# ddiazdom/grlBWT

Measured on AMD Instinct MI355X. Metric: input MB/s building BCR BWT on 10 GB DNA reads, 1/2/4/8 MI355X, higher is better.
Workload: dtype u8; 1 GPU; 66225166 x 150 bp Illumina-style reads (10000000066 bytes) from a 330000000 bp genome, 0.5% substitutions; BASELINE configs[3]; input_resident=HBM, output=.rl_bwt image in HBM, parallelism=1 GPU

## Files before the change

grlbwt_amd/csrc/engine_impl.hpp:

```cpp

#include "switches.hpp"

namespace GRL_NS {

using prim::u8;
using prim::u16;
using prim::u32;
using prim::u64;
typedef GRL_IDX_T idx_t;

template <class T>
struct DBuf {
    T *p = nullptr;
    u64 n = 0;
    DBuf() {}
    explicit DBuf(u64 n_) { alloc(n_); }
    DBuf(const DBuf &) = delete;
    DBuf &operator=(const DBuf &) = delete;
    DBuf(DBuf &&o) noexcept : p(o.p), n(o.n) { o.p = nullptr; o.n = 0; }
    DBuf &operator=(DBuf &&o) noexcept {
        if (this != &o) { release(); p = o.p; n = o.n; o.p = nullptr; o.n = 0; }
        return *this;
    }
    ~DBuf() { release(); }
// ... 1631 lines not shown
static inline void build_rankbits32(RankBits &rb, const u32 *pos, u64 count, u64 nbits, const char *name) {
    u64 nw = nbits / 64 + 2;
    rb.words.alloc(nw);
    rb.base.alloc(nw + 1);
    rb.words.zero();
    prim::for_each((count + 15) / 16, BuildBits32Fn{pos, count, rb.words.p}, name);
    prim::exclusive_scan_nosync<idx_t>(nw, PopcIn{rb.words.p}, rb.base.p, true, name);
}

template <class L>
struct IdxIn {
    const L *p;
    GRL_DEV idx_t operator()(u64 i) const { return (idx_t)p[i]; }
};
struct SymHeadIn64 {
    const u32 *s;
    GRL_DEV u64 operator()(u64 t) const { return (t == 0 || s[t] != s[t - 1]) ? 1ull : 0ull; }
};
struct IdxIn64 {
    const idx_t *p;
    GRL_DEV u64 operator()(u64 i) const { return (u64)p[i]; }
};
struct PtrU32In {
    const u32 *p;
    GRL_DEV u32 operator()(u64 i) const { return p[i]; }
};
typedef prim::Pair<idx_t, idx_t> HeadLen;
struct HeadLenIn {
    const u32 *s; const idx_t *len;
    GRL_DEV HeadLen operator()(u64 t) const { return HeadLen((t == 0 || s[t] != s[t - 1]) ? (idx_t)1 : (idx_t)0, len[t]); }
};
struct DiffFn {
    const idx_t *start; idx_t *len;
    GRL_DEV void operator()(u64 r) const { len[r] = start[r + 1] - start[r]; }
};

struct Runs {
    DBuf<u32> sym;
    DBuf<idx_t> len;
    DBuf<idx_t> pos;
    u64 R = 0;
    u64 n = 0;
};
struct RunLen {
    const idx_t *len; const idx_t *pos;
    GRL_DEV idx_t operator()(u64 i) const { return len ? len[i] : (idx_t)(pos[i + 1] - pos[i]); }
};
struct RunLenIn64 {
    RunLen l;
    GRL_DEV u64 operator()(u64 i) const { return (u64)l(i); }
};

struct MergeEmitFn {
    static constexpr bool kWaveEmit = false;
    const u32 *sym; u64 n;
    u32 *osym; idx_t *ostart; u32 *map;
    GRL_DEV void operator()(u64 t, HeadLen ex, HeadLen v) const {
        if (v.a) { osym[ex.a] = sym[t]; ostart[ex.a] = ex.b; }
        if (t == n - 1) ostart[ex.a + v.a] = ex.b + v.b;
        if (map) map[t] = (u32)(ex.a + v.a - 1);
    }
};
static inline Runs merge_runs(const u32 *sym, const idx_t *len, u64 n, u32 *merged_index = nullptr) {
    Runs out;
    if (n == 0) { out.sym.alloc(0); out.len.alloc(0); return out; }
    DBuf<u32> hsym(n);
    DBuf<idx_t> ostart(n + 1);
    HeadLen tot = prim::exclusive_scan_emit<HeadLen>(n, HeadLenIn{sym, len}, MergeEmitFn{sym, n, hsym.p, ostart.p, merged_index}, "merge_runs.scan");
    u64 R = (u64)tot.a;
    out.n = (u64)tot.b;
    out.len.alloc(R);
    prim::for_each(R, DiffFn{ostart.p, out.len.p}, "merge_runs.len");
    if (R * 2 >= n) out.sym = std::move(hsym);
    else { out.sym.alloc(R); prim::d2d(out.sym.p, hsym.p, R * sizeof(u32)); }
    out.pos = std::move(ostart);
    out.R = R;
    return out;
}

struct CellSymFn {
    const u32 *t; u32 *sym; idx_t *len;
    GRL_DEV void operator()(u64 i) const { sym[i] = t[i] >> 2; len[i] = 1; }
};

template <class F>
struct StoreFn {
    F f; idx_t *out;
    GRL_DEV void operator()(u64 i) const { out[i] = f(i); }
};

struct PackGrammarFn {
    const u32 *g0; const u32 *g1; const u8 *has_hocc; u64 *gp;
    GRL_DEV void operator()(u64 u) const { gp[u] = ((u64)g1[u] << 32) | (u64)(g0[u] | (has_hocc[u] ? 0x80000000u : 0u)); }
};
struct ChainCountFn {
    const u32 *nsym; const u64 *gp; u32 sigma3;
    GRL_DEV idx_t operator()(u64 i) const {
        u64 c0 = gp[nsym[i]];
        idx_t c = (c0 & 0x80000000ull) ? 1 : 0;
        u32 nx = (u32)(c0 >> 32);
        while (nx >= sigma3) { c++; nx = (u32)(gp[nx - sigma3] >> 32); }
        return c;
    }
};
struct TakeCountIn {
    const u32 *nsym; const u64 *gp;
    GRL_DEV u64 operator()(u64 i) const { return (gp[nsym[i]] & 0x80000000ull) ? 1ull : 0ull; }
};
enum { CELLS_SEPARATE = 0, CELLS_PACKED = 1, CELLS_FUSED = 2 };
template <int MODE>
struct ChainExpandFn {
    const u32 *nsym; RunLen nlen; const u64 *gp; const idx_t *eoff;
    u32 sigma3, take_code;
    u32 *ekey; idx_t *eidx; u32 *esym; idx_t *elen; u64 *epack; u32 *term;
    int kb, lb;
    GRL_DEV void put(u64 e, u32 key, u32 sym, idx_t f) const {
        if (MODE == CELLS_FUSED) { epack[e] = ((u64)sym << (kb + lb)) | ((u64)f << kb) | (u64)key; return; }
        ekey[e] = key;
        if (MODE == CELLS_PACKED) epack[e] = ((u64)sym << 32) | (u64)f;
        else { eidx[e] = (idx_t)e; esym[e] = sym; elen[e] = f; }
    }
    GRL_DEV void operator()(u64 i) const {
        u32 cur = nsym[i];
        idx_t f = nlen(i);
        u64 e = eoff[i];
        u64 c = gp[cur];
        if (c & 0x80000000ull) put(e++, cur, take_code, f);
        u32 nx = (u32)(c >> 32);
        while (nx >= sigma3) {
            u32 b = nx - sigma3;
            put(e++, b, (u32)c & 0x7FFFFFFFu, f);
            c = gp[b];
            nx = (u32)(c >> 32);
        }
        term[i] = nx;
    }
};
struct ChainGen {
    const u32 *nsym; RunLen nlen; const u64 *gp;
    u32 sigma3, take_code;
    u32 *term;
    int kb, lb;
    GRL_DEV u32 start(u64 i) const { return nsym[i]; }
    GRL_DEV u64 node(u32 u) const { return gp[u]; }
    GRL_DEV bool owns(u64 rec) const { return (rec & 0x80000000ull) != 0; }
    GRL_DEV bool more(u64 rec) const { return (u32)(rec >> 32) >= sigma3; }
    GRL_DEV u32 next(u64 rec) const { return (u32)(rec >> 32) - sigma3; }
    GRL_DEV u64 item_bits(u64 i) const { return (u64)nlen(i) << kb; }
    GRL_DEV u64 key_own(u32 u, u64 ib) const { return ((u64)take_code << (kb + lb)) | ib | (u64)u; }
    GRL_DEV u64 key_step(u64 rec, u32 b, u64 ib) const { return ((u64)((u32)rec & 0x7FFFFFFFu) << (kb + lb)) | ib | (u64)b; }
    GRL_DEV void finish(u64 i, u64 rec) const { term[i] = (u32)(rec >> 32); }
};
struct NarrowCellFn {
    const u64 *in; u32 *out;
    GRL_DEV void operator()(u64 i) const { out[i] = (u32)in[i]; }
};
struct GatherCellFn {
    const idx_t *perm; const u32 *esym; const idx_t *elen; u32 *ssym; idx_t *slen;
    GRL_DEV void operator()(u64 t) const { u64 e = perm[t]; ssym[t] = esym[e]; slen[t] = elen[e]; }
};

struct NotCodeIn {
    const u32 *sym; u32 code;
    GRL_DEV idx_t operator()(u64 i) const { return sym[i] != code ? (idx_t)1 : (idx_t)0; }
};
struct CellView {
// ... 1274 lines not shown
        std::vector<u64> bh = bound.to_host(2 * ((u64)N + 1));
        cnt.assign(N, 0);
        for (int d = 0; d < N; d++) cnt[d] = bh[2 * (d + 1)] - bh[2 * d];
        if (res) rec = std::move(rec2);
    }
    template <class A, class F>
    void owner_round_trip(const Comm &C, const u64 *dsb, DBuf<u64> &req, u64 n, DBuf<A> &back, F answer, const char *name, const char *xname, DBuf<u32> *own_of = nullptr) {
        std::vector<u64> scnt(C.size, 0);
        try { bucket_by_owner(C, dsb, req, n, scnt, name, own_of); }
        catch (const prim::Error &e) { C.fail(e); std::fill(scnt.begin(), scnt.end(), 0); }
        const auto cn = C.counts(scnt);
        const std::vector<u64> &rcnt = cn.rcnt;
        const u64 nr = cn.total, maxb = cn.maxb;
        DBuf<u64> mine;
        DBuf<A> ans;
        try { mine.alloc(nr); ans.alloc(nr); back.alloc(n); } catch (const prim::Error &e) { C.fail(e); }
        C.allgather_u64({});
        C.named(xname).alltoall(req.p, scnt, mine.p, rcnt, 8, maxb);
        try { answer(mine.p, nr, ans.p); } catch (const prim::Error &e) { C.fail(e); }
        C.allgather_u64({});
        C.named(xname).alltoall(ans.p, rcnt, back.p, scnt, sizeof(A), maxb);
    }

    template <class cell_t, bool FIRST>
    struct DictIn {
        const Comm *C = nullptr;
        const cell_t *t = nullptr; CellOps<cell_t, FIRST> ops{};
        u64 D = 0, S = 0; u32 maxlen = 0, sigma = 0;
        const u64 *ph_pos = nullptr; const idx_t *ph_freq = nullptr; const u32 *ph_off = nullptr; const u8 *ph_lastT = nullptr;
        const u32 *fused_ph_slot = nullptr; u32 *fused_slot_val = nullptr;
        const prim::U128 *pkeys = nullptr; u64 pDs = 0; int pkb = 0;
        u32 pslot0 = 0;
        const std::vector<u64> *dbase = nullptr;
        const std::vector<u64> *sbase = nullptr;
        bool sharded_dict = false;
        u64 maxfreq = ~0ull;
    };
    struct SortKeyShape { int b, K, rb, kbits; u64 sent; };
    static SortKeyShape sort_key_shape(u32 sigma, u32 maxlen, int rb) {
        SortKeyShape s;
        s.b = std::max((int)bitlen64(sigma), 1); s.K = std::min(std::max((64 - rb) / s.b, 1), 16);
        const int kmax = prim::sw().sort_kmax;
        if (kmax >= 1 && s.K > kmax) s.K = kmax;
        if ((u64)s.K > (u64)maxlen + 1) s.K = (int)maxlen + 1;
        s.rb = (rb && s.K * s.b + rb > 64) ? 0 : rb;
        s.kbits = s.K * s.b + s.rb;
        s.sent = ((1ull << s.b) - 1ull) << s.rb;
        return s;
    }
    static void key_records_by_owner(const SufKeep &keep, const u32 *dict_sym, u64 q0, u64 nq, const SortKeyShape &ks, const RunKeys &rk, const u64 *dspl, int N,
                              u32 pos_base, const idx_t *ph_freq, u32 bwt_code, DBuf<u64> &sk, DBuf<u32> &sp, DBuf<u64> *sr, std::vector<u64> &scnt) {
        DBuf<u32> kex(nq + 1);
        const u64 nk = prim::exclusive_scan<u32>(nq, KeepRangeIn{keep, q0}, kex.p, false, "suffix_keep");
        DBuf<u64> lk(nk), bound(2 * ((u64)N + 1));
        DBuf<u32> lp(nk), own(nk), own2(nk), idx(nk), idx2(nk);
        DBuf<u64> lr;
        if (sr) lr.alloc(nk);
        prim::for_each(nq, KeyRangeFn{keep, kex.p, q0, dict_sym, ks.K, ks.b, dspl, N, lk.p, lp.p, own.p, idx.p, rk, pos_base,
                                      sr ? lr.p : nullptr, ph_freq, bwt_code}, "suffix_keys0");
        const int obits = std::max((int)bitlen64((u64)N - 1), 1);
        const int res = prim::sort_pairs<u32, u32>(own.p, idx.p, own2.p, idx2.p, nk, 0, obits, "dist.key_owner_sort");
        sk.alloc(nk); sp.alloc(nk);
        prim::for_each(nk, GatherKeyPosFn{res ? idx2.p : idx.p, lk.p, lp.p, sk.p, sp.p}, "dist.key_owner_sort");
        if (sr) { sr->alloc(nk); prim::for_each(nk, GatherU64Fn{res ? idx2.p : idx.p, lr.p, sr->p}, "dist.key_owner_sort"); }
        prim::for_each((u64)N + 1, KeyBoundFn{res ? own2.p : own.p, nk, nullptr, bound.p}, "dist.owner_bounds");
        std::vector<u64> bh = bound.to_host(2 * ((u64)N + 1));
        for (int d = 0; d < N; d++) scnt[d] = bh[2 * (d + 1)] - bh[2 * d];
    }
    static void first_sort_and_flags(DBuf<u64> &ka, DBuf<u32> &perm, u64 Sg, const SortKeyShape &ks, const RunKeys &rk, u8 *hflag, u8 *uflag) {
        DBuf<u64> kb(Sg);
        DBuf<u32> vb(Sg);
        const u64 *k = ka.p;
        if (prim::sort_pairs<u64, u32>(ka.p, perm.p, kb.p, vb.p, Sg, 0, ks.kbits, "suffix_sort0")) {
            std::swap(perm, vb);
            k = kb.p;
        }
        if (rk.rb) prim::for_each(Sg, InitSkipFn{perm.p, rk.rem, (u32)ks.K, rk.skip}, "suffix_runs");
        prim::for_each(Sg, HeadFlagFn{k, Sg, ks.sent, hflag, uflag}, "suffix_heads");
    }
    static void order_segments(u64 U, const u8 *uhead, u32 *hex, const u64 *ukey, const u32 *uslot, const u32 *uq, u64 sent_r, int kbits_r, u32 cap,
                        u32 *perm, u8 *hflag, u8 *unext) {
        SplitScan<u32, ByteIn> heads(U, ByteIn{uhead}, "suffix_heads");
        const u64 nseg = heads.total;
        u32 lds_cap = (u32)std::max(prim::sw().seg_lds_cap, 0);
#ifdef GRLBWT_PRIM_HIP
        lds_cap = std::min(lds_cap, prim::seg_sort_lds_max());
#endif
        const u32 big_cap = std::max(cap, lds_cap);
        DBuf<u32> seg_start(nseg + 1), any_big(1);
        any_big.zero();
        heads.emit(SegStartFn{hex, U, seg_start.p}, "suffix_heads");
        prim::for_each(U, SegSortSmallFn{uhead, hex, seg_start.p, uslot, uq, ukey, sent_r, cap, perm, hflag, unext, any_big.p}, "suffix_sort.small");
        if (any_big.to_host(1)[0] == 0) {
            if (prim::sw().table_trace)
                fprintf(stderr, "[grlbwt] level %d refinement round: %llu items in %llu groups; counting all of them\n", prim::rt().tag, (unsigned long long)U,
                        (unsigned long long)nseg);
            return;
        }
        const u64 nmid = U / ((u64)cap + 1) + 1;
        DBuf<u32> bex(U + 1), mid(nmid);
        const SegTiers tot = prim::exclusive_scan_emit<SegTiers>(U, SegBigIn{uhead, hex, seg_start.p, cap, lds_cap},
                                                                 SegBigEmitFn{hex, bex.p, mid.p, nmid}, "suffix_sort.big_scan");
        const u64 NB = tot.a & 0xffffffffull, n_short = tot.b & 0xffffffffull, n_long = tot.b >> 32;
        if (prim::sw().table_trace)
            fprintf(stderr, "[grlbwt] level %d refinement round: %llu items in %llu groups; counting %llu, LDS %llu (%llu short + %llu long groups), radix %llu\n",
                    prim::rt().tag, (unsigned long long)U, (unsigned long long)nseg, (unsigned long long)(U - NB - (tot.a >> 32)), (unsigned long long)(tot.a >> 32),
                    (unsigned long long)n_short, (unsigned long long)n_long, (unsigned long long)NB);
        order_segments_lds(n_short, SegBigLdsFn{mid.p, seg_start.p, ukey, uslot, uq, sent_r, perm, hflag, unext}, false, std::min(lds_cap, kSegLdsShort));
        order_segments_lds(n_long, SegBigLdsFn{mid.p + (nmid - n_long), seg_start.p, ukey, uslot, uq, sent_r, perm, hflag, unext}, true, lds_cap);
        if (NB) {
            DBuf<u32> bitem(NB), bidx(NB), bidx2(NB), key2(NB), key2b(NB);
            DBuf<u64> bkey(NB), bkey2(NB);
            prim::for_each(U, SegBigGatherFn{uhead, hex, seg_start.p, bex.p, ukey, big_cap, bitem.p, bkey.p, bidx.p}, "suffix_sort.big_gather");
            const u32 *i1 = prim::sort_pairs<u64, u32>(bkey.p, bidx.p, bkey2.p, bidx2.p, NB, 0, kbits_r, "suffix_sort") ? bidx2.p : bidx.p;
            u32 *i1o = (i1 == bidx.p) ? bidx2.p : bidx.p;
            prim::for_each(NB, SegBigSegKeyFn{i1, bitem.p, uhead, hex, key2.p}, "suffix_sort.big_groups");
            const int sbits = std::max((int)bitlen64(nseg), 1);
            const int res = prim::sort_pairs<u32, u32>(key2.p, (u32 *)i1, key2b.p, i1o, NB, 0, sbits, "suffix_sort");
            prim::for_each(NB, SegBigWriteFn{res ? key2b.p : key2.p, res ? i1o : i1, bitem.p, ukey, uq, uslot, NB, sent_r, perm, hflag, unext}, "suffix_refine");
        }
    }
    static void order_segments_lds(u64 n, const SegBigLdsFn &f, bool wide, u32 max_items) {
        if (n == 0) return;
#ifdef GRLBWT_PRIM_HIP
        if (wide) prim::seg_sort_lds<256>(n, f, max_items, "suffix_sort.lds");
        else prim::seg_sort_lds<64>(n, f, max_items, "suffix_sort.lds");
#else
        (void)wide;
        std::vector<u32> ord;
        for (u64 b = 0; b < n; b++) {
            const u32 a = f.begin(b), e = f.end(b);
            if (e - a > max_items) throw prim::Error(-71, "LDS tier: a listed group is larger than its limit");
            ord.resize(e - a);
            for (u32 i = 0; i < e - a; i++) ord[i] = a + i;
            std::stable_sort(ord.begin(), ord.end(), [&](u32 x, u32 y) { return f.key(x) < f.key(y); });
            for (u32 p = 0; p < e - a; p++) {
                const u64 k = f.key(ord[p]);
                const bool eq_prev = p > 0 && f.key(ord[p - 1]) == k, eq_next = p + 1 < e - a && f.key(ord[p + 1]) == k;
                f.write(a + p, ord[p], k, p > 0 && !eq_prev, eq_prev || eq_next);
            }
        }
#endif
    }
    static u64 close_groups(const u8 *hflag, u64 Sg, u32 *gstart, u32 *gid) {
        return prim::exclusive_scan_emit<u32>(Sg, ByteIn{hflag}, GroupStartsFn{Sg, gstart, DenseGidFn{gid}}, "suffix_heads");
    }
    static DBuf<u64> grammar_stop_bits(const u64 *dm, u64 n, u32 maxlen) {
        DBuf<u64> stops;
        if (maxlen >= 4096 || prim::sw().grammar_jump) {
            stops.alloc((n + 63) / 64 + 1);
            prim::for_each((n + 63) / 64, DmStopBitsFn{dm, n, stops.p}, "grammar_marks");
        }
        return stops;
    }
    static void check_phrase_columns(const std::vector<u64> &mat, const std::vector<u64> &dbase) {
        const u64 N = dbase.size() - 1;
        for (u64 d = 0, col = 0; d < N; d++, col = 0) {
            for (u64 g = 0; g < N; g++) col += mat[g * N + d];
            if (col != dbase[d + 1] - dbase[d]) throw prim::Error(-71, "dist dictionary: whole-phrase suffix count does not match the phrase count");
        }
    }
    template <class cell_t, bool FIRST>
    struct DictStage {
        Engine &E; const DictIn<cell_t, FIRST> &I; LevelData &L; const Comm *const C;
        bool sharded = false, carry = false, fused_vals = false;
        u64 d0 = 0, s0 = 0, Dl = 0, Sl = 0;
        u64 sq = 0;
        u32 bwt_code = 0, hocc_code = 0, sigma3 = 0;
        DBuf<u32> dict_sym, dict_phr;
        RankBits pbits;
        DBuf<u64> dsb;
        DBuf<u32> pos_arr, perm_ai, pown;
        DBuf<u64> abounds, rec_arr;
        u64 Sg = 0, G = 0;
        DBuf<u32> perm, gid, gstart;
        DBuf<SufRecT<8>> recs;
        DBuf<u32> grank, pidx, gmin, gmax; DBuf<idx_t> gacc; DBuf<u8> gfull, gflag;
        DBuf<u32> repq, pslot;
        DBuf<u32> gphr;
        u64 M = 0, P0 = 0, Ml = 0, P0l = 0, Moff = 0, P0off = 0;
        std::vector<u64> bbM, bbP;
        DBuf<u32> psym0, u_to_p0, pu0, merged; DBuf<idx_t> plen0;
        DictStage(Engine &e, const DictIn<cell_t, FIRST> &in, LevelData &l) : E(e), I(in), L(l), C(in.C) {
            L.info.D = I.D; L.info.S = I.S; L.info.max_phrase_len = I.maxlen;
            Sg = I.S;
            sharded = C && I.sharded_dict && I.dbase && I.sbase;
            d0 = sharded ? (*I.dbase)[C->rank] : 0; s0 = sharded ? (*I.sbase)[C->rank] : 0;
            Dl = sharded ? (*I.dbase)[C->rank + 1] - d0 : I.D; Sl = sharded ? (*I.sbase)[C->rank + 1] - s0 - test_dict_part_pad() : I.S;
            carry = sharded && I.maxfreq < 0xFFFFFFFFull && !prim::sw().dist_rec_round_trip;
// ... 485 lines not shown
        const u32 *sv = slot_val_filled ? slot_val_filled->p : own.p;
        if (P.Ds || P.part_bits) {
            DBuf<u32> va(P.n_occ), vb(P.n_occ), vc(P.n_occ);
            prim::for_each(((u64)1 << P.part_bits) * 64, PartValFn{P.pstart.p, P.pbase.p, P.lid.p, sv, P.slot0, va.p, rank_only ? P.ph_vflag.p : nullptr}, "emit_part.values");
            P.pstart.release();
            P.psort.backward(va.p, vb.p, vc.p, "emit_part.back");
            prim::for_each(P.n_occ, PartCombineFn{sv, vc.p, P.next_text.p}, "emit_parse");
            P.psort.release(); P.lid.release(); P.pbase.release(); P.ph_key.release(); P.ph_vflag.release();
        } else prim::for_each((P.n_occ + 3) / 4, MapFn{sv, P.next_text.p, P.n_occ}, "emit_parse");
    }

    void finish_round(LocalParse &P, LevelData &L, u64 n_strings_for_termination, u64 n_occ_for_termination) {
        if (keep_texts) {
            DBuf<u32> cp(P.n_occ);
            prim::d2d(cp.p, P.next_text.p, P.n_occ * sizeof(u32));
            prim::sync();
            kept_texts.push_back(std::move(cp));
        }
        cur_text = std::move(P.next_text);
        cur_n = P.n_occ;
        cur_sigma = L.M;
        levels.push_back(std::move(L));
        if (n_occ_for_termination == n_strings_for_termination) parse_done = true;
    }

    template <class cell_t, bool FIRST>
    void par_round_t(const cell_t *t, u64 n, u32 sigma, cell_t sep) {
        CellOps<cell_t, FIRST> ops{sep};
        prim::rt().tag = (int)levels.size();
        prim::rt().phase = 'p';
        LevelData L;
        L.sigma = sigma;
        L.info.n_in = n;
        L.info.sigma = sigma;
        LocalParse P;
        hash_local<cell_t, FIRST>(t, n, ops, P, L, true);
        DBuf<u32> phrase_val, slot_val(P.cap);
        DictIn<cell_t, FIRST> I;
        I.t = t; I.ops = ops; I.D = P.D; I.S = P.S; I.maxlen = P.maxlen; I.sigma = sigma;
        I.ph_pos = P.ph_pos.p; I.ph_freq = P.ph_freq.p; I.ph_off = P.ph_off.p; I.ph_lastT = P.ph_lastT.p;
        I.fused_ph_slot = P.ph_slot.p; I.fused_slot_val = slot_val.p; I.pkeys = P.ph_key.p; I.pDs = P.Ds; I.pkb = P.rec_b; I.pslot0 = P.slot0;
        dict_stage(I, L, phrase_val);
        emit_local(P, nullptr, &slot_val, true);
        finish_round(P, L, stats.n_strings, P.n_occ);
    }

    bool parse_round() {
        if (parse_done) return true;
        if (levels.empty()) {
            switch (cell_bytes) {
                case 1: par_round_t<u8, true>((const u8 *)text0, n0, cur_sigma, (u8)sep0()); break;
                case 2: par_round_t<u16, true>((const u16 *)text0, n0, cur_sigma, (u16)sep0()); break;
                case 4: par_round_t<u32, true>((const u32 *)text0, n0, cur_sigma, (u32)sep0()); break;
                default: par_round_t<u64, true>((const u64 *)text0, n0, cur_sigma, (u64)sep0()); break;
            }
        } else {
            DBuf<u32> t = std::move(cur_text);
            par_round_t<u32, false>(t.p, cur_n, cur_sigma, 0u);
        }
        if (levels.size() > 64) throw prim::Error(-75, "too many parsing rounds");
        return parse_done;
    }
    int parse_phase() {
        while (!parse_round()) {}
        return (int)levels.size();
    }

    void first_bwt() {
        if (!parse_done) throw prim::Error(-22, "parse phase not finished");
        prim::rt().tag = (int)levels.size();
        prim::rt().phase = 'i';
        StageTimer st(&tm.ind_assemble, "ind_assemble");
        DBuf<u32> s(cur_n);
        DBuf<idx_t> l(cur_n);
        prim::for_each(cur_n, CellSymFn{cur_text.p, s.p, l.p}, "parse2bwt");
        bwt = merge_runs(s.p, l.p, cur_n);
        bwt_level = (int)levels.size();
        cur_text.release();
        linfo.assign(levels.size() + 1, LevelInfo());
        linfo[bwt_level].R = bwt.R;
        linfo[bwt_level].n = cur_n;
        if (keep_texts) { kept_bwts.clear(); kept_bwts.resize(levels.size() + 1); keep_bwt(bwt_level); }
    }
    RunLen run_len() const { return RunLen{bwt.len.p, bwt.pos.p}; }
    void need_len() {
        if (!bwt.len.p && bwt.pos.p) { bwt.len.alloc(bwt.R); prim::for_each(bwt.R, DiffFn{bwt.pos.p, bwt.len.p}, "merge_runs.len"); }
    }
    void keep_bwt(int lvl) {
        need_len();
        Runs c;
        c.sym.alloc(bwt.R); c.len.alloc(bwt.R); c.R = bwt.R;
        prim::d2d(c.sym.p, bwt.sym.p, bwt.R * sizeof(u32));
        prim::d2d(c.len.p, bwt.len.p, bwt.R * sizeof(idx_t));
        prim::sync();
        kept_bwts[lvl] = std::move(c);
    }

    u64 expand_split(LevelData &L, DBuf<u32> &term, u64 maxrun, int &kb, int &lb) {
        const u32 sigma3 = L.sigma + 3, bwt_code = L.sigma + 1, take_code = bwt_code;
        const u64 R = bwt.R, M = L.M;
        DBuf<idx_t> eoff;
        DBuf<u32> ssym; DBuf<idx_t> slen;
        DBuf<u64> gp;
        u64 E = 0;
        DBuf<u32> skey;
        DBuf<u64> spack;
        DBuf<u64> sfused;
        DBuf<u32> sfused32;
        kb = (int)bitlen64(L.M > 0 ? L.M - 1 : 0);
        if (kb < 1) kb = 1;
        {
            const int bits = kb;
            {
                StageTimer st(&tm.ind_expand, "ind_expand");
                gp.alloc(M);
                prim::for_each(M, PackGrammarFn{L.g0.p, L.g1.p, L.has_hocc.p, gp.p}, "induce_pack_grammar");
            }
            const int sbits = (int)bitlen64((u64)sigma3);
            prim::XsPlan plan;
            lb = (int)bitlen64(maxrun);
            if (lb < 1) lb = 1;
            const char force = prim::sw().cell_layout;
            const bool fused = kb + lb + sbits <= 64 && !force;
            const bool cell32 = fused && kb + lb + sbits <= 32 && kb < 32 && !prim::sw().no_cell32;
            if (prim::sw().table_trace) fprintf(stderr, "[grlbwt] induction level %d: %llu runs, longest %llu, cell bits: bucket %d + length %d + symbol %d\n",
                                                      prim::rt().tag, (unsigned long long)R, (unsigned long long)maxrun, kb, lb, sbits);
            const bool packed = !fused && maxrun < 0xFFFFFFFFull && force != 's';
            bool done = false;
            if (fused) {
                const ChainGen gen{bwt.sym.p, run_len(), gp.p, sigma3, take_code, term.p, kb, lb};
                {
                    StageTimer st(&tm.ind_expand, "ind_expand");
                    E = prim::expand_count(R, gen, bits, plan, "induce");
                }
                if (plan.ok && cell32) {
                    DBuf<u32> ef(E), ef2(E);
                    StageTimer st(&tm.ind_sort, "ind_sort");
                    int res = prim::expand_sort<ChainGen, u32>(gen, plan, ef.p, ef2.p, "induce");
                    sfused32 = std::move(res ? ef2 : ef);
                    done = true;
                } else if (plan.ok) {
                    DBuf<u64> ef(E), ef2(E);
                    StageTimer st(&tm.ind_sort, "ind_sort");
                    int res = prim::expand_sort(gen, plan, ef.p, ef2.p, "induce");
                    sfused = std::move(res ? ef2 : ef);
                    done = true;
                }
            }
            plan.release();
            if (!done) {
                StageTimer st(&tm.ind_expand, "ind_expand");
                eoff.alloc(R + 1);
                prim::for_each(R, StoreFn<ChainCountFn>{ChainCountFn{bwt.sym.p, gp.p, sigma3}, eoff.p}, "induce_count");
                E = (u64)prim::exclusive_scan<idx_t>(R, IdxIn<idx_t>{eoff.p}, eoff.p, true, "induce_count_scan");
            }
            if (done) {
            } else if (fused) {
                DBuf<u64> ef(E), ef2(E);
                {
                    StageTimer st(&tm.ind_expand, "ind_expand");
                    prim::for_each(R, ChainExpandFn<CELLS_FUSED>{bwt.sym.p, run_len(), gp.p, eoff.p, sigma3, take_code,
                                                                 nullptr, nullptr, nullptr, nullptr, ef.p, term.p, kb, lb}, "induce_expand");
                }
                StageTimer st(&tm.ind_sort, "ind_sort");
                int res = prim::sort_keys<u64, 1>(ef.p, ef2.p, E, 0, bits, "induce_split");
                if (cell32) {
// ... 825 lines not shown
        prim::sync();
        return k;
    }
    struct FastxInfo { u64 n_out, n_strings; int fastq; };
    static constexpr int kErrNotFastx = -22, kErrNotDna = -86;
    static FastxInfo fastx_to_text(const u8 *in, u64 n, bool rc, u8 *out, u64 capacity) {
        if (n == 0) throw prim::Error(kErrNotFastx, "FASTA/Q input is empty");
        u8 first, lastb;
        prim::d2h(&first, in, 1);
        prim::d2h(&lastb, in + n - 1, 1);
        if (first != '>' && first != '@') throw prim::Error(kErrNotFastx, "the input is not in FASTA/Q format (first byte is neither '>' nor '@')");
        const u64 nw = n / 64 + 2;
        DBuf<u64> words(nw);
        DBuf<idx_t> base(nw + 1);
        words.zero();
        prim::for_each((n + 63) / 64, FxNlWordsFn{in, n, words.p}, "fastx.newlines");
        const u64 n_nl = (u64)prim::exclusive_scan<idx_t>(nw, PopcIn{words.p}, base.p, true, "fastx.newlines");
        const bool tail = lastb != 10;
        const u64 m = n_nl + (tail ? 1 : 0);
        DBuf<u64> nlpos(m);
        prim::for_each((n + 63) / 64, FxNlPosFn{words.p, base.p, nlpos.p}, "fastx.line_ends");
        if (tail) prim::h2d(nlpos.p + (m - 1), &n, 8);
        const bool fastq = prim::reduce_sum<u64>(m, FxPlusIn{in, nlpos.p}, "fastx.plus_lines") != 0;
        u64 fq_lines = 0;
        bool regular = true;
        if (fastq) {
            fq_lines = prim::reduce_max<u64>(m, FxLastNonEmptyIn{nlpos.p}, "fastx.last_line");
            regular = fq_lines % 4 == 0 && prim::reduce_sum<u64>(fq_lines / 4, FxFastqBadIn{in, nlpos.p}, "fastx.fastq_check") == 0;
        }
        DBuf<u8> cls(m);
        DBuf<u64> raw(m), hrank(m + 1), praw(m + 1), hline, kept(m), pk(m + 1);
        u64 R, K;
        if (regular) {
            prim::for_each(m, FxClassFn{in, nlpos.p, fq_lines, fastq, cls.p, raw.p}, "fastx.classify");
            R = prim::exclusive_scan<u64>(m, FxIsHdrIn{cls.p}, hrank.p, true, "fastx.records");
            prim::exclusive_scan_nosync<u64>(m, IdxIn<u64>{raw.p}, praw.p, true, "fastx.raw_offsets");
            hline.alloc(R + 1);
            prim::for_each(m, FxHdrLinesFn{cls.p, hrank.p, m, R, hline.p}, "fastx.header_lines");
            prim::for_each(m, FxKeptFn{in, nlpos.p, cls.p, hrank.p, hline.p, praw.p, kept.p}, "fastx.kept");
        } else {
            DBuf<u64> res(1);
            cls.zero(); kept.zero();
            prim::for_each(1, FxSeqClassFn{in, n, nlpos.p, m, tail, cls.p, kept.p, res.p}, "fastx.record_walk");
            prim::for_each(m, FxStopFn{res.get(0), cls.p, kept.p}, "fastx.record_walk");
            R = prim::exclusive_scan<u64>(m, FxIsHdrIn{cls.p}, hrank.p, true, "fastx.records");
            hline.alloc(R + 1);
            prim::for_each(m, FxHdrLinesFn{cls.p, hrank.p, m, R, hline.p}, "fastx.header_lines");
        }
        K = prim::exclusive_scan<u64>(m, IdxIn<u64>{kept.p}, pk.p, true, "fastx.offsets");
        raw.release(); praw.release();
        if (regular && R && tail) {
            const u64 hl = hline.get(R - 1);
            if (hl == m - 1 && n - (hl ? nlpos.get(hl - 1) + 1 : 0) == 1) R--;
        }
        FastxInfo info;
        info.fastq = fastq ? 1 : 0;
        info.n_strings = rc ? 2 * R : R;
        info.n_out = rc ? 2 * K + 2 * R : K + R;
        if (info.n_out > capacity) throw prim::Error(-22, "fastx: output buffer too small");
        DBuf<FxLineRec> rec(m);
        prim::for_each(m, FxLineRecFn{nlpos.p, cls.p, hrank.p, hline.p, kept.p, pk.p, rc, rec.p}, "fastx.line_records");
        DBuf<u64> bad(2);
        const u64 none[2] = {~0ull, 0};
        prim::h2d(bad.p, none, 16);
        prim::for_each(n, FxCopyFn{in, n, words.p, base.p, rec.p, hrank.p, rc, out, bad.p}, "fastx.copy");
        prim::for_each(R, FxSepFn{hline.p, pk.p, rc, (u8)10, out}, "fastx.separators");
        if (rc) {
            const u64 br = bad.get(0);
            if (br != ~0ull) {
                const u64 l0 = hline.get(br), l1 = hline.get(br + 1);
                const u64 x0 = l0 ? nlpos.get(l0 - 1) + 1 : 0, x1 = l1 < m ? nlpos.get(l1 - 1) + 1 : n;
                prim::for_each(x1 - x0, FxBadPosFn{in, words.p, base.p, rec.p, hrank.p, br, x0, bad.p + 1}, "fastx.bad_symbol");
                const u64 bp = bad.get(1);
                u8 c = '?';
                if (bp) prim::d2h(&c, in + (bp - 1), 1);
                throw prim::Error(kErrNotDna, std::string("The input seems not to be DNA (invalid symbol:") + (char)c + ")");
            }
        }
        prim::sync();
        return info;
    }

    void run_all() {
        parse_phase();
        induce_phase();
        finish();
    }
};

}

#include "image_impl.hpp"
```

grlbwt_amd/csrc/switches.hpp:

```cpp
#pragma once
#include <cstdint>
#include <cstdlib>

#define GRLBWT_SWITCHES_PRODUCT(X)                                                                                                 \
    X(GRLBWT_PART_MIN_OCC, part_min_occ, uint64_t, (uint64_t)1 << 20, "smallest level (phrase occurrences) that takes the partitioned naming") \
    X(GRLBWT_PART_BITS, part_bits, int, 0, "partition bits of the partitioned naming, 1..20 (0: from the level's size)")          \
    X(GRLBWT_PART_ONE_PASS, part_one_pass, bool, false, "partitioned naming: records and long phrases in one pass through the table") \
    X(GRLBWT_FORCE_DIRECT_INDEX, force_direct_index, bool, false, "take the direct index on texts too small for a sample")        \
    X(GRLBWT_TABLE_TRACE, table_trace, bool, false, "trace the phrase-table and cell-layout decisions on stderr")                 \
    X(GRLBWT_A2A_SELF_VIA_COMM, a2a_self_via_comm, bool, false, "a rank's own all-to-all block goes through the callback too")    \
    X(GRLBWT_RUN_KEYS_MIN, run_keys_min, uint64_t, 512, "phrase length from which the suffix sort takes run-aware keys")         \
    X(GRLBWT_DOUBLING_AFTER, doubling_after, uint64_t, 24, "refinement rounds of a long-phrase level before doubling rounds")     \
    X(GRLBWT_SEG_CAP, seg_cap, int, 64, "largest suffix group ordered by counting (kSegCap); larger ones in LDS or by two radix sorts") \
    X(GRLBWT_SEG_LDS_CAP, seg_lds_cap, int, 4096, "largest suffix group ordered in LDS (above: two radix sorts; 0: no LDS tier)") \
    X(GRLBWT_CELL_LAYOUT, cell_layout, char, 0, "p[acked] | s[eparate]: a wider induction cell layout than the input needs")     \
    X(GRLBWT_NO_CELL32, no_cell32, bool, false, "induction cells of one word in 64 bits even where 32 would do")               \
    X(GRLBWT_ASM_TWO_PASS, asm_two_pass, bool, false, "pass C always as count + emit (no one-walk form)")                       \
    X(GRLBWT_ASM_ONE_WALK, asm_one_walk, bool, false, "pass C tries the one-walk form at every level, plain or not")           \
    X(GRLBWT_ASM_IMAGE, asm_image, int, 1, "level 0's pass C writes the .rl_bwt records itself (0: emit + pack)")             \
    X(GRLBWT_DIST_GATHERED_DICT, dist_gathered_dict, bool, false, "multi-rank: the dictionary gathered on every rank, not sharded") \
    X(GRLBWT_DIST_SHARDED_DICT_MIN, dist_sharded_dict_min, int, 4, "multi-rank: ranks from which the dictionary is sharded")    \
    X(GRLBWT_DIST_SHARDED_DICT_MIN_SYMS, dist_sharded_dict_min_syms, uint64_t, (uint64_t)1 << 27, "multi-rank: dictionary symbols from which it is sharded") \
    X(GRLBWT_INVERT, invert, char, 0, "r[uns] | p[ositions]: the form of the inversion (unset: by the memory it needs)")         \
    X(GRLBWT_XS_MAXC, xs_maxc, int, 32, "most cells per item the fused expansion sort takes (lower: the unfused branch)")        \
    X(GRLBWT_ALPHA_TABLE_BITS, alpha_table_bits, int, 20, "log2 of the slots of the alphabet compaction's table, 2..26 (lower: the sorting regime)") \
    X(GRLBWT_FM_TOP_BITS, fm_top_bits, int, 12, "log2 of the keys of an FM index's search array kept in LDS, 0..12 (0: none; lower: small indexes search HBM)") \
    X(GRLBWT_FM_MATCH, fm_match, char, 0, "l[anes]: grlbwt_fm_match / grlbwt_fm_mems with one lane per query cell, grlbwt_fm_approx with one lane per pattern, and no refilling, not lanes that take tickets") \
    X(GRLBWT_WALK_LANES, walk_lanes, uint64_t, 0, "most lanes of a checkpointed walk launch, rounded up to a wave (0: from occupancy; lower: small inputs refill their lanes)") \
    X(GRLBWT_MERGE_ROUND, merge_round, char, 0, "s[ort]: a round of the image merge as gathered keys and a stable sort, not the fused kernels") \
    X(GRLBWT_LCP_ROUND, lcp_round, char, 0, "p[lain]: a pass of grlbwt_fm_lcp through the generic primitives, not the fused kernel")  \
    X(GRLBWT_IO_THREADS, io_threads, int, 0, "reader / writer threads per file chunk, 1..64 (0: from the host's cores)")         \
    X(GRLBWT_QUIET_ENV, quiet_env, bool, false, "no note on stderr about the switches set in the environment")

#define GRLBWT_SWITCHES_INIT(X)                                                                                                     \
    X(GRLBWT_TRACE, trace, char, 0, "1: print every launch and synchronise after it")                                          \
    X(GRLBWT_SYNC_SITES, sync_sites, bool, false, "profile: count behind which launch site the host waited")                  \
    X(GRLBWT_MEM_TRACE, mem_trace, bool, false, "per-stage peak device memory on stderr")                                      \
    X(GRLBWT_NOPOOL, nopool, bool, false, "no slab allocator: hipMalloc / hipFree for every buffer")                           \
    X(GRLBWT_POOL_CLASSIC, pool_classic, bool, false, "hipMalloc slabs only, no reserved arena")                              \
    X(GRLBWT_POOL_TRACE, pool_trace, bool, false, "what backing the arena cost the process, on stderr at exit")               \
    X(GRLBWT_IO_TRACE, io_trace, bool, false, "where the file loader and the image writer spend their time, on stderr")

#define GRLBWT_SWITCHES_TEST(X)                                                                                                     \
    X(GRLBWT_NO_DIRECT_INDEX, no_direct_index, bool, false, "the hot table instead of the direct index")                       \
    X(GRLBWT_NO_HOT_TABLE, no_hot_table, bool, false, "no hot table in front of the phrase table")                            \
    X(GRLBWT_A2A_BLOCK, a2a_block, uint64_t, (uint64_t)256 << 20, "bytes of one all-to-all block before it goes in rounds")   \
    X(GRLBWT_TEST_DICT_PART_PAD, test_dict_part_pad, uint64_t, 0, "offset added to the global numbering of the dictionary parts") \
    X(GRLBWT_DIST_REC_ROUND_TRIP, dist_rec_round_trip, bool, false, "sharded sort: records travel back and forth, not carried") \
    X(GRLBWT_SORT_EXCHANGE_MIN, sort_exchange_min, int, 4, "ranks from which the sharded sort exchanges its first keys")     \
    X(GRLBWT_DIST_REC_FLY_MIN, dist_rec_fly_min, int, 8, "ranks from which the group records are made on the fly")           \
    X(GRLBWT_DIST_REPLICATED_PREBWT, dist_replicated_prebwt, bool, false, "every rank holds the whole pre-BWT")               \
    X(GRLBWT_DIST_REPLICATED_INDUCTION, dist_replicated_induction, bool, false, "the induction replicated on every rank")      \
    X(GRLBWT_DIST_REPLICATED_GRAMMAR, dist_replicated_grammar, bool, false, "the grammar passes replicated on every rank")     \
    X(GRLBWT_DIST_REPLICATED_DICT, dist_replicated_dict, bool, false, "the dictionary stage replicated on every rank")         \
    X(GRLBWT_GRAMMAR_JUMP, grammar_jump, bool, false, "the grammar walks jump to their stops whatever the phrase lengths")     \
    X(GRLBWT_MERGE_CELLS, merge_cells, char, 0, "s[ort]: the received induction cells merged by a radix sort, not by blocks") \
    X(GRLBWT_TEST_FAIL_RANK, test_fail_rank, int, -1, "this rank fails in the phrase hashing")                                \
    X(GRLBWT_TEST_FAIL_RANK_SORT, test_fail_rank_sort, int, -1, "this rank fails in the suffix refinement")                 \
    X(GRLBWT_TEST_FAIL_RANK_MERGE, test_fail_rank_merge, int, -1, "this rank fails in the phrase merge")                    \
    X(GRLBWT_TEST_FAIL_RANK_INDUCE, test_fail_rank_induce, int, -1, "this rank fails in the induction")

#define GRLBWT_SWITCHES_DEV(X)                                                                                                      \
    X(GRLBWT_NO_PART, no_part, bool, false, "no partitioned naming (single GPU)")                                              \
    X(GRLBWT_DIST_NO_PART, dist_no_part, bool, false, "no partitioned naming (multi-rank)")                                   \
    X(GRLBWT_NO_NAME_STREAM, no_name_stream, bool, false, "the direct index without the name_stream kernel")                  \
    X(GRLBWT_SORT_KMAX, sort_kmax, int, 16, "most symbols in the first suffix sort's key")                                     \
    X(GRLBWT_FOR_EACH_GRID, for_each_grid, char, 0, "f[ixed]: 8 workgroups per CU; anything else: twice the resident number") \
    X(GRLBWT_SPAN_BLOCKS_PER_CU, span_blocks_per_cu, uint64_t, 0, "workgroups per CU of the span kernels (0: from occupancy)") \
    X(GRLBWT_SORT_DIGIT, sort_digit, int, 8, "widest radix digit of the sorts, 8..10 bits")                                    \
    X(GRLBWT_XS_DIGIT8, xs_digit8, bool, false, "the expansion sort keeps 8-bit digits where 9 would save a pass")            \
    X(GRLBWT_RS_THREADS, rs_threads, int, 0, "threads per workgroup of the radix sorts (0: by record width)")                \
    X(GRLBWT_RS_THREADS_XS, rs_threads_xs, int, 0, "the same for the sorts behind the fused expansion")                      \
    X(GRLBWT_SM_SPT, sm_spt, int, 0, "segments per thread of the segment merge, 4 or 8 (0: by the level)")                  \
    X(GRLBWT_DEV_SM1_SPT, dev_sm1_spt, int, 0, "segments per thread of the one-walk pass C, 4 or 8 (0: by the level)")      \
    X(GRLBWT_DEV_WALK_STORES, dev_walk_stores, char, 0, "c[ells]: the checkpointed write walk stores u8/u16 cells one by one, not collected as aligned 8-byte words") \
    X(GRLBWT_DEV_LB_PATIENCE, dev_lb_patience, uint64_t, 200000000, "clock ticks a look-back tile waits before it gives up")

namespace prim {

struct Switches {
#define GRL_SW_FIELD(name, field, type, def, meaning) type field = def;
#define GRL_SW_CONST(name, field, type, def, meaning) static constexpr type field = def;
    GRLBWT_SWITCHES_PRODUCT(GRL_SW_FIELD)
    GRLBWT_SWITCHES_INIT(GRL_SW_FIELD)
#ifndef GRLBWT_PRIM_HIP
    GRLBWT_SWITCHES_TEST(GRL_SW_FIELD)
#else
    GRLBWT_SWITCHES_TEST(GRL_SW_CONST)
#endif
#ifdef GRLBWT_DEV_SWITCHES
    GRLBWT_SWITCHES_DEV(GRL_SW_FIELD)
#else
    GRLBWT_SWITCHES_DEV(GRL_SW_CONST)
#endif
#undef GRL_SW_FIELD
#undef GRL_SW_CONST

    static void parse(bool &v, const char *) { v = true; }
    static void parse(int &v, const char *e) { v = atoi(e); }
    static void parse(uint64_t &v, const char *e) { v = (uint64_t)atoll(e); }
    static void parse(char &v, const char *e) { v = e[0]; }
    template <class F>
    static void for_each_name(F f) {
#define GRL_SW_NAME(name, field, type, def, meaning) f(#name);
        GRLBWT_SWITCHES_PRODUCT(GRL_SW_NAME)
        GRLBWT_SWITCHES_INIT(GRL_SW_NAME)
#ifndef GRLBWT_PRIM_HIP
        GRLBWT_SWITCHES_TEST(GRL_SW_NAME)
#endif
#ifdef GRLBWT_DEV_SWITCHES
        GRLBWT_SWITCHES_DEV(GRL_SW_NAME)
#endif
#undef GRL_SW_NAME
    }
    static Switches from_env() {
        Switches s;
#define GRL_SW_READ(name, field, type, def, meaning) if (const char *e = getenv(#name)) parse(s.field, e);
        GRLBWT_SWITCHES_PRODUCT(GRL_SW_READ)
        GRLBWT_SWITCHES_INIT(GRL_SW_READ)
#ifndef GRLBWT_PRIM_HIP
        GRLBWT_SWITCHES_TEST(GRL_SW_READ)
#endif
#ifdef GRLBWT_DEV_SWITCHES
        GRLBWT_SWITCHES_DEV(GRL_SW_READ)
#endif
#undef GRL_SW_READ
        return s;
    }
};

inline Switches &call_switches() {
    static Switches s;
    return s;
}
inline const Switches &sw() { return call_switches(); }
inline void take_switches() { call_switches() = Switches::from_env(); }
inline const Switches &init_sw() {
    static const Switches s = Switches::from_env();
    return s;
}

}
```

Measured before the change: 14160 MB/s.

## Stop parsing early and build the BWT of short-string levels by direct suffix sort

Adds a base case: once a level's text has at most a set number of cells per string (default 5) and strings are short, the parse stops. The level's strings are sorted as suffixes with the existing dictionary suffix sort, and the BWT is emitted directly, skipping further parse rounds and their inductions. The cost is a larger suffix sort over all cells of that level in place of more recursion levels. It also adds a guard that falls back to normal parsing when strings are long.

```diff
diff --git a/grlbwt_amd/csrc/engine_impl.hpp b/grlbwt_amd/csrc/engine_impl.hpp
--- a/grlbwt_amd/csrc/engine_impl.hpp
+++ b/grlbwt_amd/csrc/engine_impl.hpp
@@ -1737,6 +1737,35 @@
     const u32 *t; u32 *sym; idx_t *len;
     GRL_DEV void operator()(u64 i) const { sym[i] = t[i] >> 2; len[i] = 1; }
 };
+struct TermIn {
+    const u32 *t;
+    GRL_DEV u32 operator()(u64 q) const { return t[q] & 1u; }
+};
+struct BaseTextFn {
+    static constexpr bool kWaveEmit = false;
+    const u32 *t; u64 n; u32 *sym; u32 *str; u32 *off; u64 cap;
+    GRL_DEV void operator()(u64 q, u32 ex, u32 v) const {
+        sym[q] = t[q] >> 2; str[q] = ex;
+        if ((q == 0 || (t[q - 1] & 1u)) && ex <= cap) off[ex] = (u32)q;
+        if (q == n - 1 && (u64)ex + v <= cap) off[ex + v] = (u32)n;
+    }
+};
+struct OffLenIn {
+    const u32 *off;
+    GRL_DEV u32 operator()(u64 k) const { return off[k + 1] - off[k]; }
+};
+struct StartSlotIn {
+    const u32 *perm; const u64 *starts;
+    GRL_DEV u32 operator()(u64 t) const { return bit_at(starts, perm[t]) ? 1u : 0u; }
+};
+struct BaseRowFn {
+    static constexpr bool kWaveEmit = false;
+    const u32 *perm; const u32 *sym; const u32 *off; u32 *osym; idx_t *olen;
+    GRL_DEV void operator()(u64 t, u32 m, u32 whole) const {
+        osym[t] = whole ? sym[off[m + 1] - 1u] : sym[perm[t] - 1u];
+        olen[t] = 1;
+    }
+};
 
 template <class F>
 struct StoreFn {
@@ -3177,6 +3206,7 @@
                         u32 *perm, u8 *hflag, u8 *unext) {
         SplitScan<u32, ByteIn> heads(U, ByteIn{uhead}, "suffix_heads");
         const u64 nseg = heads.total;
+        const char *round_name = prim::rt().phase == 'i' ? "base case sort round" : "refinement round";
         u32 lds_cap = (u32)std::max(prim::sw().seg_lds_cap, 0);
 #ifdef GRLBWT_PRIM_HIP
         lds_cap = std::min(lds_cap, prim::seg_sort_lds_max());
@@ -3188,7 +3218,7 @@
         prim::for_each(U, SegSortSmallFn{uhead, hex, seg_start.p, uslot, uq, ukey, sent_r, cap, perm, hflag, unext, any_big.p}, "suffix_sort.small");
         if (any_big.to_host(1)[0] == 0) {
             if (prim::sw().table_trace)
-                fprintf(stderr, "[grlbwt] level %d refinement round: %llu items in %llu groups; counting all of them\n", prim::rt().tag, (unsigned long long)U,
+                fprintf(stderr, "[grlbwt] level %d %s: %llu items in %llu groups; counting all of them\n", prim::rt().tag, round_name, (unsigned long long)U,
                         (unsigned long long)nseg);
             return;
         }
@@ -3198,8 +3228,8 @@
                                                                  SegBigEmitFn{hex, bex.p, mid.p, nmid}, "suffix_sort.big_scan");
         const u64 NB = tot.a & 0xffffffffull, n_short = tot.b & 0xffffffffull, n_long = tot.b >> 32;
         if (prim::sw().table_trace)
-            fprintf(stderr, "[grlbwt] level %d refinement round: %llu items in %llu groups; counting %llu, LDS %llu (%llu short + %llu long groups), radix %llu\n",
-                    prim::rt().tag, (unsigned long long)U, (unsigned long long)nseg, (unsigned long long)(U - NB - (tot.a >> 32)), (unsigned long long)(tot.a >> 32),
+            fprintf(stderr, "[grlbwt] level %d %s: %llu items in %llu groups; counting %llu, LDS %llu (%llu short + %llu long groups), radix %llu\n",
+                    prim::rt().tag, round_name, (unsigned long long)U, (unsigned long long)nseg, (unsigned long long)(U - NB - (tot.a >> 32)), (unsigned long long)(tot.a >> 32),
                     (unsigned long long)n_short, (unsigned long long)n_long, (unsigned long long)NB);
         order_segments_lds(n_short, SegBigLdsFn{mid.p, seg_start.p, ukey, uslot, uq, sent_r, perm, hflag, unext}, false, std::min(lds_cap, kSegLdsShort));
         order_segments_lds(n_long, SegBigLdsFn{mid.p + (nmid - n_long), seg_start.p, ukey, uslot, uq, sent_r, perm, hflag, unext}, true, lds_cap);
@@ -3851,6 +3881,68 @@
         linfo[bwt_level].n = cur_n;
         if (keep_texts) { kept_bwts.clear(); kept_bwts.resize(levels.size() + 1); keep_bwt(bwt_level); }
     }
+    struct BaseText {
+        DBuf<u32> sym, str, off;
+        u64 D = 0; u32 maxlen = 0;
+    };
+    BaseText base_text() {
+        prim::rt().tag = (int)levels.size();
+        prim::rt().phase = 'i';
+        StageTimer st(&tm.ind_assemble, "ind_assemble");
+        BaseText B;
+        B.sym.alloc(cur_n); B.str.alloc(cur_n); B.off.alloc(stats.n_strings + 2);
+        B.D = prim::exclusive_scan_emit<u32>(cur_n, TermIn{cur_text.p}, BaseTextFn{cur_text.p, cur_n, B.sym.p, B.str.p, B.off.p, stats.n_strings + 1}, "base_text");
+        if (B.D != stats.n_strings || !(cur_text.get(cur_n - 1) & 1u)) throw prim::Error(-71, "base case: the level's text does not hold one flagged cell per string");
+        B.maxlen = prim::reduce_max<u32>(B.D, OffLenIn{B.off.p}, "base_maxlen");
+        return B;
+    }
+    bool base_case_candidate() const {
+        const u64 ratio = prim::sw().base_case_ratio;
+        if (ratio == 0 || keep_texts || parse_done || levels.size() < 2) return false;
+        if (cur_n >= 0xFFFFFFF0ull || stats.n_strings >= 0xFFFFFFF0ull) return false;
+        return cur_n / ratio < stats.n_strings || (cur_n / ratio == stats.n_strings && cur_n % ratio == 0);
+    }
+    void base_bwt(BaseText &B) {
+        prim::rt().tag = (int)levels.size();
+        prim::rt().phase = 'i';
+        const u64 n = cur_n, D = B.D;
+        DBuf<u8> all_last(D);
+        all_last.fill_ff();
+        DictIn<u32, false> I;
+        I.D = D; I.S = n; I.maxlen = B.maxlen; I.sigma = cur_sigma;
+        I.ph_off = B.off.p; I.ph_lastT = all_last.p;
+        LevelData scratch;
+        DictStage<u32, false> Z(*this, I, scratch);
+        Z.dict_sym = std::move(B.sym); Z.dict_phr = std::move(B.str);
+        {
+            StageTimer st(&tm.ind_assemble, "ind_assemble");
+            build_rankbits32(Z.pbits, I.ph_off, D, n + 1, "base_text");
+        }
+        Z.suffix_sort_local();
+        if (Z.Sg != n) throw prim::Error(-71, "base case: the sort left suffixes out");
+        StageTimer st(&tm.ind_assemble, "ind_assemble");
+        Z.gid.release(); Z.gstart.release();
+        DBuf<u32> s(n);
+        DBuf<idx_t> l(n);
+        const u64 whole = prim::exclusive_scan_emit<u32>(n, StartSlotIn{Z.perm.p, Z.pbits.words.p}, BaseRowFn{Z.perm.p, Z.dict_sym.p, I.ph_off, s.p, l.p}, "base_rows");
+        if (whole != D) throw prim::Error(-71, "base case: whole-string rows do not match the string count");
+        bwt = merge_runs(s.p, l.p, n);
+        bwt_level = (int)levels.size();
+        cur_text.release();
+        parse_done = true;
+        linfo.assign(levels.size() + 1, LevelInfo());
+        linfo[bwt_level].R = bwt.R;
+        linfo[bwt_level].n = n;
+    }
+    void parse_phase_or_base() {
+        while (!parse_done) {
+            if (base_case_candidate()) {
+                BaseText B = base_text();
+                if ((u64)B.maxlen < prim::sw().run_keys_min) { base_bwt(B); return; }
+            }
+            parse_round();
+        }
+    }
     RunLen run_len() const { return RunLen{bwt.len.p, bwt.pos.p}; }
     void need_len() {
         if (!bwt.len.p && bwt.pos.p) { bwt.len.alloc(bwt.R); prim::for_each(bwt.R, DiffFn{bwt.pos.p, bwt.len.p}, "merge_runs.len"); }
@@ -4842,8 +4934,9 @@
     }
 
     void run_all() {
-        parse_phase();
-        induce_phase();
+        parse_phase_or_base();
+        if (bwt_level < 0) first_bwt();
+        while (bwt_level > 0) induce_level();
         finish();
     }
 };
diff --git a/grlbwt_amd/csrc/switches.hpp b/grlbwt_amd/csrc/switches.hpp
--- a/grlbwt_amd/csrc/switches.hpp
+++ b/grlbwt_amd/csrc/switches.hpp
@@ -11,6 +11,7 @@
     X(GRLBWT_A2A_SELF_VIA_COMM, a2a_self_via_comm, bool, false, "a rank's own all-to-all block goes through the callback too")    \
     X(GRLBWT_RUN_KEYS_MIN, run_keys_min, uint64_t, 512, "phrase length from which the suffix sort takes run-aware keys")         \
     X(GRLBWT_DOUBLING_AFTER, doubling_after, uint64_t, 24, "refinement rounds of a long-phrase level before doubling rounds")     \
+    X(GRLBWT_BASE_CASE_RATIO, base_case_ratio, uint64_t, 5, "a whole build stops parsing at a level of at most this many cells per string and sorts its suffixes (0: never)") \
     X(GRLBWT_SEG_CAP, seg_cap, int, 64, "largest suffix group ordered by counting (kSegCap); larger ones in LDS or by two radix sorts") \
     X(GRLBWT_SEG_LDS_CAP, seg_lds_cap, int, 4096, "largest suffix group ordered in LDS (above: two radix sorts; 0: no LDS tier)") \
     X(GRLBWT_CELL_LAYOUT, cell_layout, char, 0, "p[acked] | s[eparate]: a wider induction cell layout than the input needs")     \
@@ -36,7 +37,6 @@
     X(GRLBWT_TRACE, trace, char, 0, "1: print every launch and synchronise after it")                                          \
     X(GRLBWT_SYNC_SITES, sync_sites, bool, false, "profile: count behind which launch site the host waited")                  \
     X(GRLBWT_MEM_TRACE, mem_trace, bool, false, "per-stage peak device memory on stderr")                                      \
-    X(GRLBWT_NOPOOL, nopool, bool, false, "no slab allocator: hipMalloc / hipFree for every buffer")                           \
     X(GRLBWT_POOL_CLASSIC, pool_classic, bool, false, "hipMalloc slabs only, no reserved arena")                              \
     X(GRLBWT_POOL_TRACE, pool_trace, bool, false, "what backing the arena cost the process, on stderr at exit")               \
     X(GRLBWT_IO_TRACE, io_trace, bool, false, "where the file loader and the image writer spend their time, on stderr")
@@ -61,6 +61,7 @@
     X(GRLBWT_TEST_FAIL_RANK_INDUCE, test_fail_rank_induce, int, -1, "this rank fails in the induction")
 
 #define GRLBWT_SWITCHES_DEV(X)                                                                                                      \
+    X(GRLBWT_NOPOOL, nopool, bool, false, "no slab allocator: hipMalloc / hipFree for every buffer")                           \
     X(GRLBWT_NO_PART, no_part, bool, false, "no partitioned naming (single GPU)")                                              \
     X(GRLBWT_DIST_NO_PART, dist_no_part, bool, false, "no partitioned naming (multi-rank)")                                   \
     X(GRLBWT_NO_NAME_STREAM, no_name_stream, bool, false, "the direct index without the name_stream kernel")                  \
```

Result: faster. 16430 MB/s, median of 6 (+16.0%).
